# johannesulf/nautilus

Measured on AMD Instinct MI355X. Metric: effective posterior samples/sec + |dlogZ| vs analytic, 50-dim Gaussian, higher is better.
Workload: dtype f64

## Files before the change

### nautilus_amd/csrc/nb_eval_fast.hip

```cpp
#include "nb_common.h"
#include "nb_launch.h"

#include <type_traits>

#include "nb_mlp.h"

namespace {

constexpr int FAST_MAX_GROUPS = 1024;

struct FastArgs {
  const double* blob;
  int sample;
  const nb_gd* x;
  const long long* idx;
  int m;
  int recentre;
  long long n;
  unsigned char* out_u8;
  double* out_f64;
  unsigned long long seed;
  unsigned long long offset;
  unsigned long long* counters;
  const FastGroup* groups;
  const int* totals;
  const int* dense;
  long long n_pad;
  int n_groups;
  int out_mode;
  unsigned char* st;
  int* first;
};

constexpr int FAST_B_DOUBLES =
    (NB_HT1 * NB_HT2 + NB_HT2 * NB_HT3 + NB_HT3) * NB_TILE;

typedef const void __attribute__((address_space(1))) * nbf_gptr;
typedef void __attribute__((address_space(3))) * nbf_lptr;

template <int DT, int T>
__device__ __forceinline__ void ell_eval_centre(
    const double* c, const double* tiles, int n_dim,
    const double (&xin)[T][4 * DT], int lane, int lg, double (&y)[T][4 * DT],
    double (&r2)[T]) {
  double d[T][4 * DT];
#pragma unroll
  for (int ks = 0; ks < 4 * DT; ++ks) {
    const double cv = c[4 * ks + lg];
#pragma unroll
    for (int t = 0; t < T; ++t) d[t][ks] = xin[t][ks] - cv;
  }
  double part[T];
#pragma unroll
  for (int t = 0; t < T; ++t) part[t] = 0.0;
  const int live = n_dim - 16 * (DT - 1);
  const bool small = DT > 1 && live >= 1 && live <= 4;
  const int lane4 = (lane >> 4) * 16 + (lane & 3);
#pragma unroll
  for (int ht = 0; ht < DT; ++ht) {
    if (ht == DT - 1 && small) {
      double r4[T];
#pragma unroll
      for (int t = 0; t < T; ++t) r4[t] = 0.0;
#pragma unroll
      for (int ks = 0; ks < 4 * (ht + 1) - 2; ++ks) {
        const int kt = ks >> 2, s = ks & 3;
        const double a =
            tiles[(ht * (ht + 1) / 2 + kt) * NB_TILE + s * 64 + lane4];
#pragma unroll
        for (int t = 0; t < T; ++t) r4[t] = MFMA4(a, d[t][ks], r4[t]);
      }
#pragma unroll
      for (int t = 0; t < T; ++t) {
        y[t][4 * ht] = r4[t];
        y[t][4 * ht + 1] = y[t][4 * ht + 2] = y[t][4 * ht + 3] = 0.0;
        part[t] += r4[t] * r4[t];
      }
    } else if (16 * ht < n_dim) {
      nb_d4 acc[T];
#pragma unroll
      for (int t = 0; t < T; ++t) acc[t] = nb_d4{0.0, 0.0, 0.0, 0.0};
#pragma unroll
      for (int ks = 0; ks < 4 * (ht + 1); ++ks) {
        const int kt = ks >> 2, s = ks & 3;
        const double a =
            tiles[(ht * (ht + 1) / 2 + kt) * NB_TILE + s * 64 + lane];
#pragma unroll
        for (int t = 0; t < T; ++t) acc[t] = MFMA(a, d[t][ks], acc[t]);
      }
#pragma unroll
      for (int t = 0; t < T; ++t)
#pragma unroll
        for (int r = 0; r < 4; ++r) {
          y[t][4 * ht + r] = acc[t][r];
          part[t] += acc[t][r] * acc[t][r];
        }
    } else {
#pragma unroll
      for (int t = 0; t < T; ++t)
#pragma unroll
        for (int r = 0; r < 4; ++r) y[t][4 * ht + r] = 0.0;
    }
  }
#pragma unroll
  for (int t = 0; t < T; ++t) r2[t] = lane_group_sum(part[t]);
}

template <int DT, int T>
__device__ __forceinline__ void load_points_raw(
    const nb_gd* __restrict__ x, const long long (&row_of)[T], int n_dim,
    int lane, double2 (&raw)[T][2 * DT]) {
  int lg = lane >> 4;
  asm volatile("" : "+v"(lg));
  asm volatile("" : "+s"(x));
  if ((n_dim & 1) == 0) {
#pragma unroll
    for (int t = 0; t < T; ++t) {
      const nb_gd* row = x + row_of[t] * n_dim;
#pragma unroll
      for (int j = 0; j < 2 * DT; ++j) {
        const int f = 8 * j + 2 * lg;
        raw[t][j] = *(const NB_G double2*)(row + (f < n_dim ? f : n_dim - 2));
      }
    }
  } else {
#pragma unroll
    for (int t = 0; t < T; ++t) {
      const nb_gd* row = x + row_of[t] * n_dim;
#pragma unroll
      for (int j = 0; j < 2 * DT; ++j) {
        const int f = 8 * j + 2 * lg;
        raw[t][j].x = row[f < n_dim ? f : n_dim - 1];
        raw[t][j].y = row[f + 1 < n_dim ? f + 1 : n_dim - 1];
      }
    }
  }
}

template <int DT, int T>
__device__ __forceinline__ void points_from_raw(
    const double2 (&raw)[T][2 * DT], const bool (&valid)[T], int n_dim,
    int lg, double (&xin)[T][4 * DT]) {
#pragma unroll
  for (int t = 0; t < T; ++t)
#pragma unroll
    for (int j = 0; j < 2 * DT; ++j) {
      const int f = 8 * j + 2 * lg;
      xin[t][2 * j] = (valid[t] && f < n_dim) ? raw[t][j].x : 0.0;
      xin[t][2 * j + 1] = (valid[t] && f + 1 < n_dim) ? raw[t][j].y : 0.0;
    }
}

constexpr int FAST_REGION = 38 * NB_TILE;

template <int DT, int KT1, bool BATCH>
__global__ void __launch_bounds__(512) nb_eval_fast_kernel(FastArgs a) {
  constexpr int T = 1, NW = 8, DP = 16 * DT;
  constexpr int KS1 = 4 * KT1;
  constexpr bool TWO = KT1 * NB_HT1 * NB_TILE > FAST_REGION;
  constexpr int KA = TWO ? (KT1 + 1) / 2 : KT1;
  constexpr int NT = DT * (DT + 1) / 2;
  constexpr int HEAD = 128;
  constexpr int TAIL = HEAD + NT * NB_TILE;
  constexpr int TC = (2 + 2 * DP + 127) / 128;
  constexpr int ELL_CHUNKS = 1 + 2 * NT + TC;
  static_assert(DP <= HEAD, "centre fits the head");
  static_assert(TAIL + TC * 128 <= FAST_REGION, "ellipsoid block fits a region");
  static_assert(KA * NB_HT1 * NB_TILE <= FAST_REGION, "layer-1 chunk fits");
  constexpr int NA_D = KA * NB_HT1 * NB_TILE;
  constexpr int NB1_D = (KT1 - KA) * NB_HT1 * NB_TILE;
  constexpr int NC_D = FAST_B_DOUBLES;
  extern __shared__ __attribute__((aligned(16))) double lds[];
  auto reg = [&](int i) __attribute__((always_inline)) {
    return lds + (i & 1) * FAST_REGION;
  };

  const int lane = threadIdx.x & 63;
  const int wave = __builtin_amdgcn_readfirstlane(threadIdx.x >> 6);
  const int lg = lane >> 4;
  const bool m_sample = a.sample != 0;
  const double* blob = a.blob;
  const int n_dim = (int)nb_hdr(blob, NB_H_NDIM);
  const int K = (int)nb_hdr(blob, NB_H_K);
  const bool use_cube = nb_hdr(blob, NB_H_USECUBE) != 0;
  const int ks1 = (n_dim + 1 + 3) >> 2;
  const long long net_stride = nb_hdr(blob, NB_H_NET_STRIDE);
  unsigned long long cnt_ell = 0, cnt_mlp = 0;
  long long sup = blockIdx.x;

  struct Pass {
    const double* nb;
    const double* shift;
    int E, b;
    long long base;
    int n_valid;
  };
  int* pp = (int*)(lds + 2 * FAST_REGION);
  long long n_super;
  if constexpr (BATCH) {
    if (wave == 0) {
      int run = 0;
      for (int g0 = 0; g0 < a.n_groups; g0 += 64) {
        const int g = g0 + lane;
        int v = g < a.n_groups ? (a.totals[g] + 127) >> 7 : 0;
#pragma unroll
        for (int d = 1; d < 64; d <<= 1) {
          const int u = __shfl_up(v, d);
          if (lane >= d) v += u;
        }
        if (g < a.n_groups) pp[g + 1] = run + v;
        run += __shfl(v, 63);
      }
      if (lane == 0) pp[0] = 0;
    }
    __syncthreads();
    n_super = pp[a.n_groups];
    if (sup >= n_super) return;
  } else {
    n_super = (a.n + 16 * NW * T - 1) / (16 * NW * T);
  }
  auto pass_of = [&](long long P) __attribute__((always_inline)) {
    Pass ps;
    if constexpr (BATCH) {
      const long long Pc = P < n_super ? P : n_super - 1;
      int lo = 0, hi = a.n_groups;
      while (hi - lo > 1) {
        const int mid = (lo + hi) >> 1;
        if (pp[mid] <= (int)Pc) lo = mid; else hi = mid;
      }
      const int g = __builtin_amdgcn_readfirstlane(lo);
      const FastGroup gd = a.groups[g];
      ps.nb = gd.nb;
      ps.shift = a.recentre != 0 ? gd.shift : nullptr;
      ps.E = gd.E;
      ps.b = gd.b;
      const int s0 = ((int)Pc - __builtin_amdgcn_readfirstlane(pp[g])) << 7;
      ps.base = (long long)g * a.n_pad + s0;
      const int left = a.totals[g] - s0;
      ps.n_valid = P < n_super ? (left < 128 ? left : 128) : 0;
    } else {
      ps.nb = blob + nb_hdr(blob, NB_H_OFF_NEURAL) +
              a.m * nb_hdr(blob, NB_H_NEURAL_STRIDE);
      ps.shift = (a.recentre != 0 && nb_hdr(blob, NB_H_OFF_SHIFT) != 0)
                     ? blob + nb_hdr(blob, NB_H_OFF_SHIFT) : nullptr;
      ps.E = (int)nb_hdr(blob, NB_H_E);
      ps.b = 0;
      ps.base = 0;
      ps.n_valid = 0;
    }
    return ps;
  };
  Pass cur_p = pass_of(sup);

  const double* dma_src = nullptr;
  double* dma_dst = nullptr;
  int dma_c = 0, dma_n = 0;
  bool dma_ell = false;
  auto dma_begin = [&](const double* src, double* dst, int n_doubles)
      __attribute__((always_inline)) {
    dma_src = src; dma_dst = dst; dma_c = wave; dma_n = n_doubles >> 7;
    dma_ell = false;
  };
  auto dma_begin_ell = [&](const double* nb_blk, double* dst)
      __attribute__((always_inline)) {
    dma_src = nb_blk; dma_dst = dst; dma_c = wave;
    dma_n = ELL_CHUNKS;
    dma_ell = true;
  };
  auto dma_one = [&]() __attribute__((always_inline)) {
    int s_off, d_off;
    if (!dma_ell) {
      s_off = d_off = dma_c * 128;
    } else if (dma_c < 1) {
      s_off = 2 + 2 * DP;
      d_off = 0;
    } else if (dma_c < 1 + 2 * NT) {
      const int p = (dma_c - 1) >> 1, half = (dma_c - 1) & 1;
      int ht = 0;
      while ((ht + 1) * (ht + 2) / 2 <= p) ++ht;
      const int kt = p - ht * (ht + 1) / 2;
      s_off = 2 + 3 * DP + (kt * DT + ht) * NB_TILE + half * 128;
      d_off = HEAD + p * NB_TILE + half * 128;
    } else {
      const int i = dma_c - 1 - 2 * NT;
      s_off = nb_ell_block_size(DT) + i * 128;
      d_off = TAIL + i * 128;
    }
    __builtin_amdgcn_global_load_lds(
        (nbf_gptr)(dma_src + s_off + 2 * lane),
        (nbf_lptr)(dma_dst + d_off), 16, 0, 0);
    dma_c += NW;
  };
  auto dma_tick = [&]() __attribute__((always_inline)) {
    if (dma_c < dma_n) dma_one();
  };
  auto dma_flush = [&]() __attribute__((always_inline)) {
    while (dma_c < dma_n) dma_one();
  };

  int q = 0;
  dma_begin_ell(cur_p.nb, reg(0));
  dma_flush();
  long long pt[T];
  bool valid[T];
  double2 xraw[T][2 * DT];
  auto row_of = [&](long long p) __attribute__((always_inline)) {
    return p < a.n ? (a.idx != nullptr ? a.idx[p] : p) : 0ll;
  };
  auto row_in = [&](const Pass& ps, int t) __attribute__((always_inline)) {
    const int slot = (wave * T + t) * 16 + (lane & 15);
    return (long long)a.dense[ps.base + (slot < ps.n_valid ? slot : 0)];
  };
  long long nrow[T];
#pragma unroll
  for (int t = 0; t < T; ++t) {
    pt[t] = ((sup * NW + wave) * T + t) * 16 + (lane & 15);
    valid[t] = pt[t] < a.n;
    if constexpr (BATCH) nrow[t] = row_in(cur_p, t);
    else nrow[t] = row_of(pt[t]);
  }
  load_points_raw<DT, T>(a.x, nrow, n_dim, lane, xraw);

  for (; sup < n_super; sup += gridDim.x) {
    const double* nb_m = cur_p.nb;
    const double* shift = cur_p.shift;
    const int E = cur_p.E;
    const double* nets = nb_m + nb_ell_block_size(DT) + 2 + 2 * DP;
    const Pass next_p = pass_of(sup + gridDim.x);
    int lgp = lg;
    asm volatile("" : "+v"(lgp));
    long long crow[T];
    dma_begin(nets, reg(q ^ 1), NA_D);
    dma_flush();
    asm volatile("s_waitcnt vmcnt(%0)" ::"n"((NA_D / 128 + NW - 1) / NW)
                 : "memory");
    __syncthreads();
    const double* blk = reg(q);
    const double thr = blk[TAIL];

    bool in_cube[T], acc_outer[T], want[T];
    double xin[T][4 * DT];
#pragma unroll
    for (int t = 0; t < T; ++t) {
      pt[t] = ((sup * NW + wave) * T + t) * 16 + (lane & 15);
      in_cube[t] = true;
      if constexpr (BATCH) {
        valid[t] = (wave * T + t) * 16 + (lane & 15) < cur_p.n_valid;
        crow[t] = nrow[t];
        nrow[t] = row_in(next_p, t);
      } else {
        valid[t] = pt[t] < a.n;
        nrow[t] = row_of((((sup + gridDim.x) * NW + wave) * T + t) * 16 +
                         (lane & 15));
      }
    }
    points_from_raw<DT, T>(xraw, valid, n_dim, lgp, xin);
    if (shift != nullptr) {
#pragma unroll
      for (int ks = 0; ks < 4 * DT; ++ks) {
        const double sv = shift[4 * ks + lgp];
        const bool on = shift[DP + 4 * ks + lgp] != 0.0;
#pragma unroll
        for (int t = 0; t < T; ++t) {
          const double v = xin[t][ks] + sv;
          xin[t][ks] = on ? v - floor(v) : xin[t][ks];
        }
      }
    }
    if (m_sample) {
      bool cbad[T];
#pragma unroll
      for (int t = 0; t < T; ++t) cbad[t] = false;
#pragma unroll
      for (int ks = 0; ks < 4 * DT; ++ks) {
        const int f = 8 * (ks >> 1) + 2 * lgp + (ks & 1);
        const bool boxed = use_cube && f < n_dim;
#pragma unroll
        for (int t = 0; t < T; ++t)
          cbad[t] |= boxed && !(xin[t][ks] >= 0.0 && xin[t][ks] < 1.0);
      }
#pragma unroll
      for (int t = 0; t < T; ++t) {
        in_cube[t] = !point_any(cbad[t], lane);
        acc_outer[t] = in_cube[t];
        want[t] = valid[t] && acc_outer[t];
      }
    } else {
#pragma unroll
      for (int t = 0; t < T; ++t) { acc_outer[t] = false; want[t] = valid[t]; }
    }

    double y[T][4 * DT], r2[T];
    bool box_bad[T], inside_e[T], need[T];
    ell_eval_centre<DT, T>(blk, blk + HEAD, n_dim, xin, lane, lgp, y, r2);
#pragma unroll
    for (int t = 0; t < T; ++t) box_bad[t] = false;
    bool wave_mlp = false;
#pragma unroll
    for (int t = 0; t < T; ++t) {
      inside_e[t] = !box_bad[t] && r2[t] < 1.0;
      need[t] = m_sample ? (want[t] && inside_e[t]) : valid[t];
      cnt_ell += __popcll(__ballot(want[t] && lg == 0));
      cnt_mlp += (unsigned long long)E * __popcll(__ballot(need[t] && lg == 0));
      wave_mlp |= need[t];
    }
    wave_mlp = __any(wave_mlp);

    double tin[T][KS1];
    {
      const double* r_mean = blk + TAIL + 2;
      const double* r_isc = r_mean + DP;
#pragma unroll
      for (int ks = 0; ks < KS1; ++ks) {
        const int f = 4 * ks + lgp;
        if (ks < 4 * DT) {
          const double mv = r_mean[f], sv = r_isc[f];
          const double pad = (f == n_dim) ? 1.0 : 0.0;
#pragma unroll
          for (int t = 0; t < T; ++t) {
            const double v = (y[t][ks] - mv) * sv;
            tin[t][ks] = (f < n_dim) ? v : pad;
          }
        } else {
#pragma unroll
          for (int t = 0; t < T; ++t) tin[t][ks] = (f == n_dim) ? 1.0 : 0.0;
        }
      }
    }
    asm volatile("s_waitcnt vmcnt(0)" ::: "memory");
    __syncthreads();
#pragma unroll
    for (int t = 0; t < T; ++t) asm volatile("" : "+v"(nrow[t]));

    double total[T];
#pragma unroll
    for (int t = 0; t < T; ++t) total[t] = 0.0;
    int cur = q ^ 1;

    auto stage_end = [&]() __attribute__((always_inline)) {
      dma_flush();
      asm volatile("s_waitcnt vmcnt(0)" ::: "memory");
      __syncthreads();
      cur ^= 1;
    };
    auto network = [&](int e, auto last_c) __attribute__((always_inline)) {
      constexpr bool LAST = decltype(last_c)::value;
      const double* w_e = nets + e * net_stride;
      double h1[T][4 * NB_HT1];
      if constexpr (TWO) {
        dma_begin(w_e + NA_D, reg(cur ^ 1), NB1_D);
        if (wave_mlp)
          fl_chunk<T, KS1, NB_HT1, 0, 4 * KA, 2>(reg(cur), ks1, tin, lane, h1,
                                                dma_tick);
        stage_end();
        dma_begin(w_e + NA_D + NB1_D, reg(cur ^ 1), NC_D);
        if (wave_mlp) {
          fl_chunk<T, KS1, NB_HT1, 4 * KA, KS1, 1>(reg(cur), ks1, tin, lane,
                                                  h1, dma_tick);
          fl_pad<T, NB_HT1, 25, 0>(h1, lane);
        }
        stage_end();
      } else {
        dma_begin(w_e + NA_D, reg(cur ^ 1), NC_D);
        if (wave_mlp) {
          fl_chunk<T, KS1, NB_HT1, 0, KS1, 1>(reg(cur), ks1, tin, lane, h1,
                                             dma_tick);
          fl_pad<T, NB_HT1, 25, 0>(h1, lane);
        }
        stage_end();
      }
      if constexpr (LAST) {
        load_points_raw<DT, T>(a.x, nrow, n_dim, lane, xraw);
        dma_begin_ell(next_p.nb, reg(cur ^ 1));
      } else {
        dma_begin(nets + (e + 1) * net_stride, reg(cur ^ 1), NA_D);
      }
      if (wave_mlp) {
        const double* w2 = reg(cur);
        const double* w3 = w2 + NB_HT1 * NB_HT2 * NB_TILE;
        const double* w4 = w3 + NB_HT2 * NB_HT3 * NB_TILE;
        double h2[T][4 * NB_HT2], h3[T][4 * NB_HT3], o[T][4];
        double a2[FlFirst<8, NB_HT2>::NA], a3[FlFirst<8, NB_HT3>::NA],
            a4[FlFirst<8, 1>::NA];
        fl_read_first<8, NB_HT2>(w2, lane, a2);
        fl_layer_from<T, 8, 26, 0, NB_HT2, true, 2, 1, 0>(
            w2, 26, h1, lane, h2, a2,
            [&]() __attribute__((always_inline)) {
              fl_read_first<8, NB_HT3>(w3, lane, a3);
            },
            dma_tick);
        fl_pad<T, NB_HT2, 12, 2>(h2, lane);
        fl_layer_from<T, 8, 13, 0, NB_HT3, true, 2, 2, 0>(
            w3, 13, h2, lane, h3, a3,
            [&]() __attribute__((always_inline)) {
              fl_read_first<8, 1>(w4, lane, a4);
            },
            dma_tick);
        fl_pad<T, NB_HT3, 5, 0>(h3, lane);
        fl_layer_from<T, 8, 6, 0, 1, true, 2, 5, 0>(
            w4, 6, h3, lane, o, a4, []() __attribute__((always_inline)) {},
            dma_tick);
#pragma unroll
        for (int t = 0; t < T; ++t) total[t] += o[t][0];
      }
      stage_end();
    };
    for (int e = 0; e + 1 < E; ++e) network(e, std::false_type{});
    network(E - 1, std::true_type{});
    q = cur;

#pragma unroll
    for (int t = 0; t < T; ++t) {
      const double score = __shfl(total[t], lane & 15) / (double)E;
      if constexpr (BATCH) {
        if (valid[t] && lg == 0 && score > thr) {
          a.st[crow[t]] = a.out_mode == 2 ? (unsigned char)3 : (unsigned char)2;
          if (a.out_mode == 1) atomicMin(&a.first[crow[t]], cur_p.b);
        }
      } else if (m_sample) {
        bool ok = inside_e[t];
        if (need[t]) ok = inside_e[t] && (score > thr);
        const unsigned char flags =
            (acc_outer[t] ? 1 : 0) | ((acc_outer[t] && ok) ? 2 : 0);
        if (valid[t] && lg == 0) a.out_u8[pt[t]] = flags;
      } else if (valid[t] && lg == 0) {
        a.out_f64[2 * pt[t]] = r2[t];
        a.out_f64[2 * pt[t] + 1] = score;
      }
    }
    cur_p = next_p;
  }
  if (a.counters != nullptr && lane == 0) {
    atomicAdd(&a.counters[1], cnt_ell);
    atomicAdd(&a.counters[2], cnt_mlp);
  }
}

template <int DT, int KT1, bool BATCH>
int launch_fast_impl(const FastArgs& a, hipStream_t stream) {
  const size_t lds = (size_t)2 * FAST_REGION * sizeof(double) +
                     (BATCH ? (FAST_MAX_GROUPS + 1) * sizeof(int) : 0);
  static bool configured = false;
  if (!configured) {
    const hipError_t e = hipFuncSetAttribute(
        (const void*)nb_eval_fast_kernel<DT, KT1, BATCH>,
        hipFuncAttributeMaxDynamicSharedMemorySize, (int)lds);
    if (e != hipSuccess) {
      nb_set_error("hipFuncSetAttribute(%zu bytes LDS) failed: %s", lds,
                   hipGetErrorString(e));
      return NB_ERR_HIP;
    }
    configured = true;
  }
  const long long n_super = (a.n + 127) / 128;
  long long blocks = n_super < 256 ? n_super : 256;
  hipLaunchKernelGGL((nb_eval_fast_kernel<DT, KT1, BATCH>),
                     dim3((unsigned)blocks), dim3(512), lds, stream, a);
  return NB_OK;
}

template <int DT, int KT1>
int launch_fast(const FastArgs& a, hipStream_t stream) {
  return a.groups != nullptr ? launch_fast_impl<DT, KT1, true>(a, stream)
                             : launch_fast_impl<DT, KT1, false>(a, stream);
}

}

bool nb_eval_fast_eligible(int n_dim, int K, int M, int E, bool sample) {
  if (n_dim > 128 || M < 1 || E < 1) return false;
  return !sample || (K <= 1 && M == 1);
}

static int dispatch_fast(const FastArgs& a, int n_dim, hipStream_t stream) {
  const int dt = (n_dim + 15) / 16, kt1 = (n_dim + 1 + 15) / 16;
  int rc = NB_ERR_UNSUPPORTED;
  switch (4 * dt + (kt1 - dt)) {
    case 4: rc = launch_fast<1, 1>(a, stream); break;
    case 5: rc = launch_fast<1, 2>(a, stream); break;
    case 8: rc = launch_fast<2, 2>(a, stream); break;
    case 9: rc = launch_fast<2, 3>(a, stream); break;
    case 12: rc = launch_fast<3, 3>(a, stream); break;
    case 13: rc = launch_fast<3, 4>(a, stream); break;
    case 16: rc = launch_fast<4, 4>(a, stream); break;
    case 17: rc = launch_fast<4, 5>(a, stream); break;
    case 20: rc = launch_fast<5, 5>(a, stream); break;
    case 21: rc = launch_fast<5, 6>(a, stream); break;
    case 24: rc = launch_fast<6, 6>(a, stream); break;
    case 25: rc = launch_fast<6, 7>(a, stream); break;
    case 28: rc = launch_fast<7, 7>(a, stream); break;
    case 29: rc = launch_fast<7, 8>(a, stream); break;
    case 32: rc = launch_fast<8, 8>(a, stream); break;
    case 33: rc = launch_fast<8, 9>(a, stream); break;
    default:
      nb_set_error("nb_launch_eval_fast: n_dim=%d not eligible", n_dim);
      return NB_ERR_UNSUPPORTED;
  }
  if (rc != NB_OK) return rc;
  NB_HIP_CHECK(hipGetLastError());
  return NB_OK;
}

int nb_launch_eval_fast(const double* blob_dev, int n_dim, bool sample, int m,
                        int recentre, const double* x, const long long* idx,
                        long long n,
                        unsigned char* out_u8, double* out_f64,
                        unsigned long long seed, unsigned long long offset,
                        hipStream_t stream) {
  if (n <= 0) return NB_OK;
  FastArgs a = {};
  a.blob = blob_dev; a.sample = sample ? 1 : 0; a.x = (const nb_gd*)x; a.n = n;
  a.idx = idx; a.m = m; a.recentre = recentre;
  a.out_u8 = out_u8; a.out_f64 = out_f64; a.seed = seed; a.offset = offset;
  a.counters = nb_eval_counters();
  return dispatch_fast(a, n_dim, stream);
}

int nb_launch_eval_fast_batch(const double* blob0_dev, int n_dim, int recentre,
                              const double* x, const void* groups_dev,
                              int n_groups, const int* totals_dev,
                              const int* dense_dev, long long n_pad,
                              long long n_upper, int out_mode,
                              unsigned char* st, int* first,
                              hipStream_t stream) {
  if (n_upper <= 0 || n_groups <= 0) return NB_OK;
  if (n_groups > FAST_MAX_GROUPS) {
    nb_set_error("nb_launch_eval_fast_batch: %d groups (limit %d)", n_groups,
                 FAST_MAX_GROUPS);
    return NB_ERR_ARG;
  }
  FastArgs a = {};
  a.blob = blob0_dev; a.sample = 0; a.x = (const nb_gd*)x;
  a.n = n_upper + 128ll * n_groups;
  a.recentre = recentre;
  a.counters = nb_eval_counters();
  a.groups = (const FastGroup*)groups_dev; a.n_groups = n_groups;
  a.totals = totals_dev; a.dense = dense_dev; a.n_pad = n_pad;
  a.out_mode = out_mode; a.st = st; a.first = first;
  return dispatch_fast(a, n_dim, stream);
}
```

### nautilus_amd/csrc/nb_mlp.h

```cpp
#pragma once
#include "nb_tile.h"

namespace {

constexpr int fl_blk_end(int HT, int H0, int SPLIT) {
  return (HT - 1 - H0 > SPLIT) ? H0 + SPLIT : HT;
}

template <int HT, int H0, int H1>
struct FlShape {
  static constexpr int NFL = HT - 1;
  static constexpr bool REM = (H1 == HT);
  static constexpr int NF = (REM ? NFL : H1) - H0;
  static constexpr int NA = NF + (REM ? 1 : 0);
};

template <int HT, int H0, int H1>
__device__ __forceinline__ void fl_read_a(
    const double* w, int ks, int lane, double (&a)[FlShape<HT, H0, H1>::NA]) {
  using S = FlShape<HT, H0, H1>;
  const double* wk = w + (ks >> 2) * HT * NB_TILE + (ks & 3) * 64;
#pragma unroll
  for (int h = 0; h < S::NF; ++h) a[h] = wk[(H0 + h) * NB_TILE + lane];
  if constexpr (S::REM)
    a[S::NF] = wk[S::NFL * NB_TILE + (lane >> 4) * 16 + (lane & 3)];
}

template <int T, int KSMAX, int NGUARD, int HT, int H0, int H1, bool RELU_IN,
          int TICK_P, int PD, int NIN, int NOUT, class Next, class Tick>
__device__ __forceinline__ void fl_block(
    const double* w, int ks_n, const double (&in)[T][NIN], int lane,
    double (&out)[T][NOUT], const double (&a0)[FlShape<HT, H0, H1>::NA],
    Next&& next, Tick&& tick) {
  using S = FlShape<HT, H0, H1>;
  constexpr int NF = S::NF, NA = S::NA, NFL = S::NFL;
  constexpr bool REM = S::REM;
  constexpr int KS_U = KSMAX - NGUARD;
  static_assert(KS_U >= 1 && KS_U >= PD && PD >= 1, "prefetch distance");
  constexpr int R = PD + 1;
  nb_d4 acc[T][NF > 0 ? NF : 1];
  double rem[T];
#pragma unroll
  for (int t = 0; t < T; ++t) {
#pragma unroll
    for (int h = 0; h < (NF > 0 ? NF : 1); ++h)
      acc[t][h] = nb_d4{0.0, 0.0, 0.0, 0.0};
    rem[t] = 0.0;
  }
  auto step = [&](int ks, const double (&a)[NA]) __attribute__((always_inline)) {
    double b[T];
#pragma unroll
    for (int t = 0; t < T; ++t)
      b[t] = RELU_IN ? fmax(in[t][ks], 0.0) : in[t][ks];
#pragma unroll
    for (int h = 0; h < NF; ++h)
#pragma unroll
      for (int t = 0; t < T; ++t) acc[t][h] = MFMA(a[h], b[t], acc[t][h]);
    if constexpr (REM) {
#pragma unroll
      for (int t = 0; t < T; ++t) rem[t] = MFMA4(a[NF], b[t], rem[t]);
    }
  };
  auto arrived = [&](const double (&a)[NA]) __attribute__((always_inline)) {
#pragma unroll
    for (int i = 0; i < NA; ++i) asm volatile("" ::"v"(a[i]));
  };
  double a[R][NA];
#pragma unroll
  for (int i = 0; i < NA; ++i) a[0][i] = a0[i];
#pragma unroll
  for (int i = 1; i < PD; ++i) fl_read_a<HT, H0, H1>(w, i, lane, a[i]);
  __builtin_amdgcn_sched_barrier(0);
#pragma unroll
  for (int ks = 0; ks < KS_U; ++ks) {
    arrived(a[ks % R]);
    __builtin_amdgcn_sched_barrier(0);
    if (ks + PD < KS_U)
      fl_read_a<HT, H0, H1>(w, ks + PD, lane, a[(ks + PD) % R]);
    else if (ks + PD == KS_U) next();
    if (ks % TICK_P == 0) tick();
    __builtin_amdgcn_sched_barrier(0);
    step(ks, a[ks % R]);
    __builtin_amdgcn_sched_barrier(0);
  }
#pragma unroll
  for (int ks = KS_U; ks < KSMAX; ++ks) {
    if (ks < ks_n) {
      double ag[NA];
      fl_read_a<HT, H0, H1>(w, ks, lane, ag);
      step(ks, ag);
    }
  }
#pragma unroll
  for (int t = 0; t < T; ++t) {
#pragma unroll
    for (int h = 0; h < NF; ++h)
#pragma unroll
      for (int r = 0; r < 4; ++r) out[t][4 * (H0 + h) + r] = acc[t][h][r];
    if constexpr (REM) out[t][4 * NFL] = rem[t];
  }
}

template <int T, int KSMAX, int HT, int KS_LO, int KS_HI, int TICK_P, int NIN,
          int NOUT, class Tick>
__device__ __forceinline__ void fl_chunk(
    const double* w, int ks_n, const double (&in)[T][NIN], int lane,
    double (&out)[T][NOUT], Tick&& tick) {
  using S = FlShape<HT, 0, HT>;
  constexpr int NF = S::NF, NA = S::NA, NFL = S::NFL;
  static_assert(KS_LO % 4 == 0 && KS_LO < KS_HI && KS_HI <= KSMAX, "chunk");
  constexpr bool FIRST = (KS_LO == 0);
  constexpr int KS_U = (KS_HI < KSMAX - 3) ? KS_HI : KSMAX - 3;
  static_assert(KS_U > KS_LO, "at least one unguarded k-step per chunk");
  nb_d4 acc[T][NF];
  double rem[T];
#pragma unroll
  for (int t = 0; t < T; ++t) {
#pragma unroll
    for (int h = 0; h < NF; ++h)
#pragma unroll
      for (int r = 0; r < 4; ++r)
        acc[t][h][r] = FIRST ? 0.0 : out[t][4 * h + r];
    rem[t] = FIRST ? 0.0 : out[t][4 * NFL];
  }
  auto step = [&](int ks, const double (&a)[NA]) __attribute__((always_inline)) {
#pragma unroll
    for (int h = 0; h < NF; ++h)
#pragma unroll
      for (int t = 0; t < T; ++t)
        acc[t][h] = MFMA(a[h], in[t][ks], acc[t][h]);
#pragma unroll
    for (int t = 0; t < T; ++t) rem[t] = MFMA4(a[NF], in[t][ks], rem[t]);
  };
  auto arrived = [&](const double (&a)[NA]) __attribute__((always_inline)) {
#pragma unroll
    for (int i = 0; i < NA; ++i) asm volatile("" ::"v"(a[i]));
  };
  double a[2][NA];
  fl_read_a<HT, 0, HT>(w, 0, lane, a[0]);
  __builtin_amdgcn_sched_barrier(0);
#pragma unroll
  for (int ks = KS_LO; ks < KS_U; ++ks) {
    const int i = ks - KS_LO;
    arrived(a[i & 1]);
    __builtin_amdgcn_sched_barrier(0);
    if (ks + 1 < KS_U) fl_read_a<HT, 0, HT>(w, i + 1, lane, a[(i + 1) & 1]);
    if (i % TICK_P == 0) tick();
    __builtin_amdgcn_sched_barrier(0);
    step(ks, a[i & 1]);
    __builtin_amdgcn_sched_barrier(0);
  }
#pragma unroll
  for (int ks = (KS_LO > KS_U ? KS_LO : KS_U); ks < KS_HI; ++ks) {
    if (ks < ks_n) {
      double ag[NA];
      fl_read_a<HT, 0, HT>(w, ks - KS_LO, lane, ag);
      step(ks, ag);
    }
  }
#pragma unroll
  for (int t = 0; t < T; ++t) {
#pragma unroll
    for (int h = 0; h < NF; ++h)
#pragma unroll
      for (int r = 0; r < 4; ++r) out[t][4 * h + r] = acc[t][h][r];
    out[t][4 * NFL] = rem[t];
  }
}

template <int T, int SPLIT, int KSMAX, int NGUARD, int HT, bool RELU_IN,
          int TICK_P, int PD, int H0, int NIN, int NOUT, class Next, class Tick>
__device__ __forceinline__ void fl_layer_from(
    const double* w, int ks_n, const double (&in)[T][NIN], int lane,
    double (&out)[T][NOUT],
    const double (&a0)[FlShape<HT, H0, fl_blk_end(HT, H0, SPLIT)>::NA],
    Next&& next, Tick&& tick) {
  constexpr int H1 = fl_blk_end(HT, H0, SPLIT);
  if constexpr (H1 < HT) {
    constexpr int H2 = fl_blk_end(HT, H1, SPLIT);
    double a1[FlShape<HT, H1, H2>::NA];
    fl_block<T, KSMAX, NGUARD, HT, H0, H1, RELU_IN, TICK_P, PD>(
        w, ks_n, in, lane, out, a0,
        [&]() __attribute__((always_inline)) {
          fl_read_a<HT, H1, H2>(w, 0, lane, a1);
        },
        tick);
    fl_layer_from<T, SPLIT, KSMAX, NGUARD, HT, RELU_IN, TICK_P, PD, H1>(
        w, ks_n, in, lane, out, a1, next, tick);
  } else {
    fl_block<T, KSMAX, NGUARD, HT, H0, HT, RELU_IN, TICK_P, PD>(
        w, ks_n, in, lane, out, a0, next, tick);
  }
}

template <int SPLIT, int HT>
struct FlFirst {
  static constexpr int H1 = fl_blk_end(HT, 0, SPLIT);
  static constexpr int NA = FlShape<HT, 0, H1>::NA;
};
template <int SPLIT, int HT>
__device__ __forceinline__ void fl_read_first(
    const double* w, int lane, double (&a)[FlFirst<SPLIT, HT>::NA]) {
  fl_read_a<HT, 0, FlFirst<SPLIT, HT>::H1>(w, 0, lane, a);
}

template <int T, int HT, int ONE_KS, int ONE_LG, int NOUT>
__device__ __forceinline__ void fl_pad(double (&out)[T][NOUT], int lane) {
#pragma unroll
  for (int t = 0; t < T; ++t)
#pragma unroll
    for (int r = 1; r < 4; ++r) {
      const int idx = 4 * (HT - 1) + r;
      out[t][idx] = (idx == ONE_KS && (lane >> 4) == ONE_LG) ? 1.0 : 0.0;
    }
  if constexpr (ONE_KS >= 0 && ONE_KS == 4 * (HT - 1)) {
    if ((lane >> 4) == ONE_LG) {
#pragma unroll
      for (int t = 0; t < T; ++t) out[t][ONE_KS] = 1.0;
    }
  }
}

}
```

Baseline: 2.596 million.

## Skip dead weight pieces in DMA and ride layer-1 weights with ellipsoid block

New measurement: 2.621 million, median of 6. No clear change (+1.0%).

```diff
diff --git a/nautilus_amd/csrc/nb_eval_fast.hip b/nautilus_amd/csrc/nb_eval_fast.hip
--- a/nautilus_amd/csrc/nb_eval_fast.hip
+++ b/nautilus_amd/csrc/nb_eval_fast.hip
@@ -30,7 +30,30 @@
   int out_mode;
   unsigned char* st;
   int* first;
+#ifdef NB_FAST_STAMPS
+  unsigned long long* stamps;
+#endif
 };
+
+#ifdef NB_FAST_STAMPS
+constexpr int FAST_STAMP_SLOTS = 64, FAST_STAMP_PASS = 2;
+enum { ST_PASS = 0, ST_TOP_LEFT, ST_PROLOGUE_DONE, ST_PROLOGUE_LEFT,
+       ST_MFMA_DONE, ST_STAGE_LEFT, ST_PASS_END };
+unsigned long long* g_fast_stamps = nullptr;
+#define FAST_STAMP(kind)                                                     \
+  do {                                                                       \
+    if (wave == 0 && stamp_pass == FAST_STAMP_PASS && a.stamps != nullptr && \
+        stamp_k < FAST_STAMP_SLOTS) {                                        \
+      const unsigned long long t_ = __builtin_amdgcn_s_memtime();            \
+      if (lane == 0)                                                         \
+        a.stamps[(long long)blockIdx.x * FAST_STAMP_SLOTS + stamp_k] =       \
+            (t_ << 4) | (unsigned long long)(kind);                          \
+      ++stamp_k;                                                             \
+    }                                                                        \
+  } while (0)
+#else
+#define FAST_STAMP(kind) do {} while (0)
+#endif
 
 constexpr int FAST_B_DOUBLES =
     (NB_HT1 * NB_HT2 + NB_HT2 * NB_HT3 + NB_HT3) * NB_TILE;
@@ -153,11 +176,55 @@
 
 constexpr int FAST_REGION = 38 * NB_TILE;
 
-template <int DT, int KT1, bool BATCH>
+constexpr bool fast_l1_tail_dead(int kt1, int n_dim) {
+  return ((n_dim + 1 + 3) >> 2) <= 4 * (kt1 - 1) + 2;
+}
+constexpr int fast_l1_live_pieces(int kt1, int n_dim) {
+  return 2 * NB_HT1 * (kt1 - 1) +
+         (fast_l1_tail_dead(kt1, n_dim) ? NB_HT1 : 2 * NB_HT1);
+}
+constexpr int FAST_KS2 = (NB_H1 + 1 + 3) / 4, FAST_KS3 = (NB_H2 + 1 + 3) / 4,
+              FAST_KS4 = (NB_H3 + 1 + 3) / 4;
+static_assert(FAST_KS2 <= 4 * (NB_HT1 - 1) + 2 &&
+                  FAST_KS3 <= 4 * (NB_HT2 - 1) + 2 &&
+                  FAST_KS4 <= 4 * (NB_HT3 - 1) + 2,
+              "second pieces of the last k-tiles of layers 2-4 are dead");
+constexpr int FAST_F2 = 2 * (NB_HT1 - 1) * NB_HT2, FAST_Q2 = NB_HT2;
+constexpr int FAST_F3 = 2 * (NB_HT2 - 1) * NB_HT3, FAST_Q3 = NB_HT3;
+constexpr int FAST_F4 = 2 * (NB_HT3 - 1), FAST_Q4 = 1;
+constexpr int FAST_P3 = 2 * NB_HT1 * NB_HT2;
+constexpr int FAST_P4 = FAST_P3 + 2 * NB_HT2 * NB_HT3;
+constexpr int FAST_C_LIVE =
+    FAST_F2 + FAST_Q2 + FAST_F3 + FAST_Q3 + FAST_F4 + FAST_Q4;
+__device__ __forceinline__ int fast_c_piece(int c) {
+  constexpr int L3 = FAST_F2 + FAST_Q2, L4 = L3 + FAST_F3 + FAST_Q3;
+  int p = c;
+  if (c >= FAST_F2) p = FAST_F2 + 2 * (c - FAST_F2);
+  if (c >= L3) p = FAST_P3 + (c - L3);
+  if (c >= L3 + FAST_F3) p = FAST_P3 + FAST_F3 + 2 * (c - L3 - FAST_F3);
+  if (c >= L4) p = FAST_P4 + (c - L4);
+  if (c >= L4 + FAST_F4) p = FAST_P4 + FAST_F4 + 2 * (c - L4 - FAST_F4);
+  return p;
+}
+
+constexpr int fast_block_doubles(int dt) {
+  return 128 + dt * (dt + 1) / 2 * NB_TILE +
+         (2 + 2 * 16 * dt + 127) / 128 * 128;
+}
+constexpr bool fast_two_chunks(int kt1) {
+  return kt1 * NB_HT1 * NB_TILE > FAST_REGION;
+}
+constexpr bool fast_l1_rides(int dt, int kt1, int n_dim) {
+  return !fast_two_chunks(kt1) &&
+         fast_block_doubles(dt) + 128 * fast_l1_live_pieces(kt1, n_dim) <=
+             FAST_REGION;
+}
+
+template <int DT, int KT1, bool RIDE, bool BATCH>
 __global__ void __launch_bounds__(512) nb_eval_fast_kernel(FastArgs a) {
   constexpr int T = 1, NW = 8, DP = 16 * DT;
   constexpr int KS1 = 4 * KT1;
-  constexpr bool TWO = KT1 * NB_HT1 * NB_TILE > FAST_REGION;
+  constexpr bool TWO = fast_two_chunks(KT1);
   constexpr int KA = TWO ? (KT1 + 1) / 2 : KT1;
   constexpr int NT = DT * (DT + 1) / 2;
   constexpr int HEAD = 128;
@@ -167,9 +234,14 @@
   static_assert(DP <= HEAD, "centre fits the head");
   static_assert(TAIL + TC * 128 <= FAST_REGION, "ellipsoid block fits a region");
   static_assert(KA * NB_HT1 * NB_TILE <= FAST_REGION, "layer-1 chunk fits");
+  static_assert(fast_block_doubles(DT) == TAIL + TC * 128, "block size");
+  static_assert(!RIDE || fast_l1_rides(DT, KT1, 16 * (KT1 - 1)),
+                "no n_dim of this instantiation rides");
+  constexpr int L1_OFF = RIDE ? TAIL + TC * 128 : 0;
   constexpr int NA_D = KA * NB_HT1 * NB_TILE;
   constexpr int NB1_D = (KT1 - KA) * NB_HT1 * NB_TILE;
-  constexpr int NC_D = FAST_B_DOUBLES;
+  static_assert(FAST_P4 + FAST_F4 + 2 * FAST_Q4 == FAST_B_DOUBLES / 128 &&
+                    FAST_B_DOUBLES <= FAST_REGION, "layers 2-4 fit a region");
   extern __shared__ __attribute__((aligned(16))) double lds[];
   auto reg = [&](int i) __attribute__((always_inline)) {
     return lds + (i & 1) * FAST_REGION;
@@ -252,25 +324,55 @@
   };
   Pass cur_p = pass_of(sup);
 
+  enum { DMA_L1 = 0, DMA_C = 1, DMA_ELL = 2 };
+  const bool l1_tail_dead = fast_l1_tail_dead(KT1, n_dim);
   const double* dma_src = nullptr;
+  const double* dma_l1_src = nullptr;
   double* dma_dst = nullptr;
-  int dma_c = 0, dma_n = 0;
-  bool dma_ell = false;
-  auto dma_begin = [&](const double* src, double* dst, int n_doubles)
+  double* dma_l1_dst = nullptr;
+  const int wave7 = wave & (NW - 1);
+  int dma_k = 0, dma_n = 0, dma_mode = DMA_L1;
+  int dma_l1_c0 = 0, dma_l1_full = 0;
+  auto dma_l1_run = [&](const double* net, double* dst, int kt0, int nkt)
       __attribute__((always_inline)) {
-    dma_src = src; dma_dst = dst; dma_c = wave; dma_n = n_doubles >> 7;
-    dma_ell = false;
+    const bool last = kt0 + nkt == KT1;
+    dma_l1_src = net + kt0 * NB_HT1 * NB_TILE;
+    dma_l1_dst = dst;
+    dma_l1_full = 2 * NB_HT1 * (nkt - (last ? 1 : 0));
+    return dma_l1_full + (last ? (l1_tail_dead ? NB_HT1 : 2 * NB_HT1) : 0);
+  };
+  auto dma_begin_l1 = [&](const double* net, double* dst, int kt0, int nkt)
+      __attribute__((always_inline)) {
+    dma_k = 0; dma_mode = DMA_L1; dma_l1_c0 = 0;
+    dma_n = dma_l1_run(net, dst, kt0, nkt);
+  };
+  auto dma_begin_c = [&](const double* src, double* dst)
+      __attribute__((always_inline)) {
+    dma_src = src; dma_dst = dst; dma_k = 0; dma_n = FAST_C_LIVE;
+    dma_mode = DMA_C;
   };
   auto dma_begin_ell = [&](const double* nb_blk, double* dst)
       __attribute__((always_inline)) {
-    dma_src = nb_blk; dma_dst = dst; dma_c = wave;
+    dma_src = nb_blk; dma_dst = dst; dma_k = 0;
     dma_n = ELL_CHUNKS;
-    dma_ell = true;
-  };
-  auto dma_one = [&]() __attribute__((always_inline)) {
+    dma_mode = DMA_ELL;
+    dma_l1_c0 = ELL_CHUNKS;
+    if constexpr (RIDE)
+      dma_n += dma_l1_run(nb_blk + nb_ell_block_size(DT) + 2 + 2 * DP,
+                          dst + L1_OFF, 0, KT1);
+  };
+  auto dma_one = [&](int dma_c) __attribute__((always_inline)) {
+    const double* src = dma_src;
+    double* dst = dma_dst;
     int s_off, d_off;
-    if (!dma_ell) {
-      s_off = d_off = dma_c * 128;
+    if (dma_mode == DMA_C) {
+      s_off = d_off = fast_c_piece(dma_c) * 128;
+    } else if (dma_mode == DMA_L1 || (RIDE && dma_c >= ELL_CHUNKS)) {
+      const int c = dma_c - dma_l1_c0, j = c - dma_l1_full;
+      const int half = j >= NB_HT1 ? 1 : 0;
+      src = dma_l1_src; dst = dma_l1_dst;
+      s_off = (j < 0 ? c : dma_l1_full + 2 * (j - NB_HT1 * half) + half) * 128;
+      d_off = c * 128;
     } else if (dma_c < 1) {
       s_off = 2 + 2 * DP;
       d_off = 0;
@@ -287,15 +389,15 @@
       d_off = TAIL + i * 128;
     }
     __builtin_amdgcn_global_load_lds(
-        (nbf_gptr)(dma_src + s_off + 2 * lane),
-        (nbf_lptr)(dma_dst + d_off), 16, 0, 0);
-    dma_c += NW;
+        (nbf_gptr)(src + s_off + 2 * lane),
+        (nbf_lptr)(dst + d_off), 16, 0, 0);
   };
   auto dma_tick = [&]() __attribute__((always_inline)) {
-    if (dma_c < dma_n) dma_one();
+    if (wave7 + NW * dma_k < dma_n) dma_one(wave7 + NW * dma_k);
+    ++dma_k;
   };
   auto dma_flush = [&]() __attribute__((always_inline)) {
-    while (dma_c < dma_n) dma_one();
+    for (; wave7 + NW * dma_k < dma_n; ++dma_k) dma_one(wave7 + NW * dma_k);
   };
 
   int q = 0;
@@ -320,8 +422,19 @@
     else nrow[t] = row_of(pt[t]);
   }
   load_points_raw<DT, T>(a.x, nrow, n_dim, lane, xraw);
-
+  if constexpr (RIDE) {
+    asm volatile("s_waitcnt vmcnt(0)" ::: "memory");
+    __syncthreads();
+  }
+
+#ifdef NB_FAST_STAMPS
+  int stamp_pass = -1, stamp_k = 0;
+#endif
   for (; sup < n_super; sup += gridDim.x) {
+#ifdef NB_FAST_STAMPS
+    ++stamp_pass;
+#endif
+    FAST_STAMP(ST_PASS);
     const double* nb_m = cur_p.nb;
     const double* shift = cur_p.shift;
     const int E = cur_p.E;
@@ -330,11 +443,21 @@
     int lgp = lg;
     asm volatile("" : "+v"(lgp));
     long long crow[T];
-    dma_begin(nets, reg(q ^ 1), NA_D);
-    dma_flush();
-    asm volatile("s_waitcnt vmcnt(%0)" ::"n"((NA_D / 128 + NW - 1) / NW)
-                 : "memory");
-    __syncthreads();
+    if constexpr (!RIDE) {
+      dma_begin_l1(nets, reg(q ^ 1), 0, KA);
+      dma_flush();
+      constexpr int FULL_A = 2 * NB_HT1 * (TWO ? KA : KT1 - 1);
+      if (TWO)
+        asm volatile("s_waitcnt vmcnt(%0)" ::"n"(FULL_A / NW) : "memory");
+      else if (l1_tail_dead)
+        asm volatile("s_waitcnt vmcnt(%0)" ::"n"((FULL_A + NB_HT1) / NW)
+                     : "memory");
+      else
+        asm volatile("s_waitcnt vmcnt(%0)" ::"n"((FULL_A + 2 * NB_HT1) / NW)
+                     : "memory");
+      __syncthreads();
+      FAST_STAMP(ST_TOP_LEFT);
+    }
     const double* blk = reg(q);
     const double thr = blk[TAIL];
 
@@ -427,20 +550,26 @@
         }
       }
     }
-    asm volatile("s_waitcnt vmcnt(0)" ::: "memory");
-    __syncthreads();
+    FAST_STAMP(ST_PROLOGUE_DONE);
+    if constexpr (!RIDE) {
+      asm volatile("s_waitcnt vmcnt(0)" ::: "memory");
+      __syncthreads();
+      FAST_STAMP(ST_PROLOGUE_LEFT);
+    }
 #pragma unroll
     for (int t = 0; t < T; ++t) asm volatile("" : "+v"(nrow[t]));
 
     double total[T];
 #pragma unroll
     for (int t = 0; t < T; ++t) total[t] = 0.0;
-    int cur = q ^ 1;
+    int cur = RIDE ? q : q ^ 1;
 
     auto stage_end = [&]() __attribute__((always_inline)) {
+      FAST_STAMP(ST_MFMA_DONE);
       dma_flush();
       asm volatile("s_waitcnt vmcnt(0)" ::: "memory");
       __syncthreads();
+      FAST_STAMP(ST_STAGE_LEFT);
       cur ^= 1;
     };
     auto network = [&](int e, auto last_c) __attribute__((always_inline)) {
@@ -448,23 +577,23 @@
       const double* w_e = nets + e * net_stride;
       double h1[T][4 * NB_HT1];
       if constexpr (TWO) {
-        dma_begin(w_e + NA_D, reg(cur ^ 1), NB1_D);
+        dma_begin_l1(w_e, reg(cur ^ 1), KA, KT1 - KA);
         if (wave_mlp)
-          fl_chunk<T, KS1, NB_HT1, 0, 4 * KA, 2>(reg(cur), ks1, tin, lane, h1,
-                                                dma_tick);
+          fl_chunk<T, KS1, NB_HT1, 0, 4 * KA, 2, -1>(reg(cur), ks1, tin, lane,
+                                                    h1, dma_tick);
         stage_end();
-        dma_begin(w_e + NA_D + NB1_D, reg(cur ^ 1), NC_D);
+        dma_begin_c(w_e + NA_D + NB1_D, reg(cur ^ 1));
         if (wave_mlp) {
-          fl_chunk<T, KS1, NB_HT1, 4 * KA, KS1, 1>(reg(cur), ks1, tin, lane,
-                                                  h1, dma_tick);
+          fl_chunk<T, KS1, NB_HT1, 4 * KA, KS1, 1, KT1 - KA - 1>(
+              reg(cur), ks1, tin, lane, h1, dma_tick);
           fl_pad<T, NB_HT1, 25, 0>(h1, lane);
         }
         stage_end();
       } else {
-        dma_begin(w_e + NA_D, reg(cur ^ 1), NC_D);
+        dma_begin_c(w_e + NA_D, reg(cur ^ 1));
         if (wave_mlp) {
-          fl_chunk<T, KS1, NB_HT1, 0, KS1, 1>(reg(cur), ks1, tin, lane, h1,
-                                             dma_tick);
+          fl_chunk<T, KS1, NB_HT1, 0, KS1, 1, KT1 - 1>(
+              reg(cur) + L1_OFF, ks1, tin, lane, h1, dma_tick);
           fl_pad<T, NB_HT1, 25, 0>(h1, lane);
         }
         stage_end();
@@ -473,7 +602,8 @@
         load_points_raw<DT, T>(a.x, nrow, n_dim, lane, xraw);
         dma_begin_ell(next_p.nb, reg(cur ^ 1));
       } else {
-        dma_begin(nets + (e + 1) * net_stride, reg(cur ^ 1), NA_D);
+        dma_begin_l1(nets + (e + 1) * net_stride, reg(cur ^ 1) + L1_OFF, 0,
+                     KA);
       }
       if (wave_mlp) {
         const double* w2 = reg(cur);
@@ -528,6 +658,7 @@
         a.out_f64[2 * pt[t] + 1] = score;
       }
     }
+    FAST_STAMP(ST_PASS_END);
     cur_p = next_p;
   }
   if (a.counters != nullptr && lane == 0) {
@@ -536,14 +667,14 @@
   }
 }
 
-template <int DT, int KT1, bool BATCH>
+template <int DT, int KT1, bool RIDE, bool BATCH>
 int launch_fast_impl(const FastArgs& a, hipStream_t stream) {
   const size_t lds = (size_t)2 * FAST_REGION * sizeof(double) +
                      (BATCH ? (FAST_MAX_GROUPS + 1) * sizeof(int) : 0);
   static bool configured = false;
   if (!configured) {
     const hipError_t e = hipFuncSetAttribute(
-        (const void*)nb_eval_fast_kernel<DT, KT1, BATCH>,
+        (const void*)nb_eval_fast_kernel<DT, KT1, RIDE, BATCH>,
         hipFuncAttributeMaxDynamicSharedMemorySize, (int)lds);
     if (e != hipSuccess) {
       nb_set_error("hipFuncSetAttribute(%zu bytes LDS) failed: %s", lds,
@@ -554,15 +685,33 @@
   }
   const long long n_super = (a.n + 127) / 128;
   long long blocks = n_super < 256 ? n_super : 256;
-  hipLaunchKernelGGL((nb_eval_fast_kernel<DT, KT1, BATCH>),
+  hipLaunchKernelGGL((nb_eval_fast_kernel<DT, KT1, RIDE, BATCH>),
                      dim3((unsigned)blocks), dim3(512), lds, stream, a);
   return NB_OK;
 }
 
+template <int DT, int KT1, bool RIDE>
+int launch_fast_ride(const FastArgs& a, hipStream_t stream) {
+  return a.groups != nullptr
+             ? launch_fast_impl<DT, KT1, RIDE, true>(a, stream)
+             : launch_fast_impl<DT, KT1, RIDE, false>(a, stream);
+}
+
 template <int DT, int KT1>
-int launch_fast(const FastArgs& a, hipStream_t stream) {
-  return a.groups != nullptr ? launch_fast_impl<DT, KT1, true>(a, stream)
-                             : launch_fast_impl<DT, KT1, false>(a, stream);
+int launch_fast(const FastArgs& a, int n_dim, hipStream_t stream) {
+  constexpr int LO = KT1 > DT ? 16 * DT : 16 * (DT - 1) + 1;
+  constexpr int HI = KT1 > DT ? 16 * DT : 16 * DT - 1;
+#ifdef NB_FAST_NO_RIDE
+  return launch_fast_ride<DT, KT1, false>(a, stream);
+#endif
+  if constexpr (fast_l1_rides(DT, KT1, HI))
+    return launch_fast_ride<DT, KT1, true>(a, stream);
+  else if constexpr (!fast_l1_rides(DT, KT1, LO))
+    return launch_fast_ride<DT, KT1, false>(a, stream);
+  else
+    return fast_l1_rides(DT, KT1, n_dim)
+               ? launch_fast_ride<DT, KT1, true>(a, stream)
+               : launch_fast_ride<DT, KT1, false>(a, stream);
 }
 
 }
@@ -576,22 +725,22 @@
   const int dt = (n_dim + 15) / 16, kt1 = (n_dim + 1 + 15) / 16;
   int rc = NB_ERR_UNSUPPORTED;
   switch (4 * dt + (kt1 - dt)) {
-    case 4: rc = launch_fast<1, 1>(a, stream); break;
-    case 5: rc = launch_fast<1, 2>(a, stream); break;
-    case 8: rc = launch_fast<2, 2>(a, stream); break;
-    case 9: rc = launch_fast<2, 3>(a, stream); break;
-    case 12: rc = launch_fast<3, 3>(a, stream); break;
-    case 13: rc = launch_fast<3, 4>(a, stream); break;
-    case 16: rc = launch_fast<4, 4>(a, stream); break;
-    case 17: rc = launch_fast<4, 5>(a, stream); break;
-    case 20: rc = launch_fast<5, 5>(a, stream); break;
-    case 21: rc = launch_fast<5, 6>(a, stream); break;
-    case 24: rc = launch_fast<6, 6>(a, stream); break;
-    case 25: rc = launch_fast<6, 7>(a, stream); break;
-    case 28: rc = launch_fast<7, 7>(a, stream); break;
-    case 29: rc = launch_fast<7, 8>(a, stream); break;
-    case 32: rc = launch_fast<8, 8>(a, stream); break;
-    case 33: rc = launch_fast<8, 9>(a, stream); break;
+    case 4: rc = launch_fast<1, 1>(a, n_dim, stream); break;
+    case 5: rc = launch_fast<1, 2>(a, n_dim, stream); break;
+    case 8: rc = launch_fast<2, 2>(a, n_dim, stream); break;
+    case 9: rc = launch_fast<2, 3>(a, n_dim, stream); break;
+    case 12: rc = launch_fast<3, 3>(a, n_dim, stream); break;
+    case 13: rc = launch_fast<3, 4>(a, n_dim, stream); break;
+    case 16: rc = launch_fast<4, 4>(a, n_dim, stream); break;
+    case 17: rc = launch_fast<4, 5>(a, n_dim, stream); break;
+    case 20: rc = launch_fast<5, 5>(a, n_dim, stream); break;
+    case 21: rc = launch_fast<5, 6>(a, n_dim, stream); break;
+    case 24: rc = launch_fast<6, 6>(a, n_dim, stream); break;
+    case 25: rc = launch_fast<6, 7>(a, n_dim, stream); break;
+    case 28: rc = launch_fast<7, 7>(a, n_dim, stream); break;
+    case 29: rc = launch_fast<7, 8>(a, n_dim, stream); break;
+    case 32: rc = launch_fast<8, 8>(a, n_dim, stream); break;
+    case 33: rc = launch_fast<8, 9>(a, n_dim, stream); break;
     default:
       nb_set_error("nb_launch_eval_fast: n_dim=%d not eligible", n_dim);
       return NB_ERR_UNSUPPORTED;
@@ -613,8 +762,17 @@
   a.idx = idx; a.m = m; a.recentre = recentre;
   a.out_u8 = out_u8; a.out_f64 = out_f64; a.seed = seed; a.offset = offset;
   a.counters = nb_eval_counters();
+#ifdef NB_FAST_STAMPS
+  a.stamps = g_fast_stamps;
+#endif
   return dispatch_fast(a, n_dim, stream);
 }
+
+#ifdef NB_FAST_STAMPS
+extern "C" void nb_eval_fast_stamps(unsigned long long* dev) {
+  g_fast_stamps = dev;
+}
+#endif
 
 int nb_launch_eval_fast_batch(const double* blob0_dev, int n_dim, int recentre,
                               const double* x, const void* groups_dev,
diff --git a/nautilus_amd/csrc/nb_mlp.h b/nautilus_amd/csrc/nb_mlp.h
--- a/nautilus_amd/csrc/nb_mlp.h
+++ b/nautilus_amd/csrc/nb_mlp.h
@@ -101,13 +101,29 @@
   }
 }
 
-template <int T, int KSMAX, int HT, int KS_LO, int KS_HI, int TICK_P, int NIN,
-          int NOUT, class Tick>
+template <int HT, int KT_SPLIT>
+__device__ __forceinline__ void fl_read_chunk(const double* w, int ks, int lane,
+                                              double (&a)[HT]) {
+  if ((ks >> 2) != KT_SPLIT) {
+    fl_read_a<HT, 0, HT>(w, ks, lane, a);
+  } else {
+    const double* wk = w + (ks >> 2) * HT * NB_TILE +
+                       ((ks >> 1) & 1) * HT * (NB_TILE / 2) + (ks & 1) * 64;
+#pragma unroll
+    for (int h = 0; h < HT - 1; ++h) a[h] = wk[h * (NB_TILE / 2) + lane];
+    a[HT - 1] =
+        wk[(HT - 1) * (NB_TILE / 2) + (lane >> 4) * 16 + (lane & 3)];
+  }
+}
+
+template <int T, int KSMAX, int HT, int KS_LO, int KS_HI, int TICK_P,
+          int KT_SPLIT, int NIN, int NOUT, class Tick>
 __device__ __forceinline__ void fl_chunk(
     const double* w, int ks_n, const double (&in)[T][NIN], int lane,
     double (&out)[T][NOUT], Tick&& tick) {
   using S = FlShape<HT, 0, HT>;
   constexpr int NF = S::NF, NA = S::NA, NFL = S::NFL;
+  static_assert(NA == HT, "layer chunk: all tiles of the layer");
   static_assert(KS_LO % 4 == 0 && KS_LO < KS_HI && KS_HI <= KSMAX, "chunk");
   constexpr bool FIRST = (KS_LO == 0);
   constexpr int KS_U = (KS_HI < KSMAX - 3) ? KS_HI : KSMAX - 3;
@@ -137,14 +153,15 @@
     for (int i = 0; i < NA; ++i) asm volatile("" ::"v"(a[i]));
   };
   double a[2][NA];
-  fl_read_a<HT, 0, HT>(w, 0, lane, a[0]);
+  fl_read_chunk<HT, KT_SPLIT>(w, 0, lane, a[0]);
   __builtin_amdgcn_sched_barrier(0);
 #pragma unroll
   for (int ks = KS_LO; ks < KS_U; ++ks) {
     const int i = ks - KS_LO;
     arrived(a[i & 1]);
     __builtin_amdgcn_sched_barrier(0);
-    if (ks + 1 < KS_U) fl_read_a<HT, 0, HT>(w, i + 1, lane, a[(i + 1) & 1]);
+    if (ks + 1 < KS_U)
+      fl_read_chunk<HT, KT_SPLIT>(w, i + 1, lane, a[(i + 1) & 1]);
     if (i % TICK_P == 0) tick();
     __builtin_amdgcn_sched_barrier(0);
     step(ks, a[i & 1]);
@@ -154,7 +171,7 @@
   for (int ks = (KS_LO > KS_U ? KS_LO : KS_U); ks < KS_HI; ++ks) {
     if (ks < ks_n) {
       double ag[NA];
-      fl_read_a<HT, 0, HT>(w, ks - KS_LO, lane, ag);
+      fl_read_chunk<HT, KT_SPLIT>(w, ks - KS_LO, lane, ag);
       step(ks, ag);
     }
   }
```
